# josebeo2016/SCL-Deepfake-audio-detection

Hardware: AMD Instinct MI355X
Metric: train-step utterances/sec (64000-sample clips) (higher is better)
Workload: dtype bf16

## Files before the change

### scl-deepfake-audio-detection_amd/csrc/gemm.hip

```cpp
#include "gemm_common.h"

using namespace sclg;

namespace {

constexpr int BM = 128, BN = 128;

struct StageK {
    __amdgpu_buffer_rsrc_t rsrc;
    unsigned rowoff[4];
    unsigned lds_off[4];
    int kcur, kend;

    __device__ __forceinline__ void init(const OpK& o, const char* base, int row0, int rowlimit, int kbegin, int kend_, int tid) {
        rsrc = make_rsrc(base);
        const int c = tid & 7;
#pragma unroll
        for (int i = 0; i < 4; ++i) {
            const int row = (tid >> 3) + 32 * i;
            const int r = row0 + row;
            rowoff[i] = r < rowlimit ? row_off(o, (unsigned)r) : OOB;
            lds_off[i] = (unsigned)(row * 128 + ((c ^ ((row >> 1) & 7)) << 4));
        }
        kcur = kbegin + 8 * c; kend = kend_;
// ... 817 lines not shown
}

extern "C" int scl_gemm_bf16(const SclGemmDesc* dp, void* stream) {
    SCL_REQUIRE(dp, "gemm: null desc");
    const SclGemmDesc& d = *dp;
    GemmK k;
    {
        const int rc = gemm_fill_k(d, k);
        if (rc != SCL_OK) return rc;
    }
    const bool at = d.flags & SCL_GEMM_A_T, bt = d.flags & SCL_GEMM_B_T;
    const bool f32ab = d.flags & SCL_GEMM_AB_F32;
    const int tiles = ((d.M + BM - 1) / BM) * ((d.N + BN - 1) / BN);
    const long long zdim = (long long)d.nb1 * d.nb2 * d.splitk;
    dim3 grid(tiles, 1, (unsigned)zdim), block(256);
    const size_t lds = 4 * TILE_BYTES;
    hipStream_t s = (hipStream_t)stream;
    if (f32ab) {
        SclProfScope prof(SCL_KID_GEMM_F32, s, 2.0 * d.M * d.N * (double)d.K * d.nb1 * d.nb2, true);
        const int rc = scl_gemm_f32_launch(d, k, s);
        if (rc != SCL_OK) return rc;
        return scl_check_launch("scl_gemm_bf16(f32 operands)");
    }
    {
        SclProfScope prof(SCL_KID_GEMM, s, 2.0 * d.M * d.N * (double)d.K * d.nb1 * d.nb2, true);
        const bool a_whole = at ? (d.M % 8 == 0) : (d.K % 8 == 0);
        const bool b_whole = bt ? (d.N % 8 == 0) : (d.K % 8 == 0);
        const bool dma = a_whole && b_whole && !(d.flags & SCL_GEMM_NO_DMA);
#ifdef SCL_EXPERIMENTS
        const long long big_tiles = (long long)((d.M + BIG_BM - 1) / BIG_BM) * ((d.N + BN - 1) / BN) * zdim;
        const bool big = dma && (d.flags & SCL_GEMM_FORCE_BIG) && !(d.flags & SCL_GEMM_NO_BIG) && d.M >= 256 && d.K >= 192 && big_tiles >= 1;
        const long long p8_tiles = (long long)((d.M + P8_BM - 1) / P8_BM) * ((d.N + P8_BN - 1) / P8_BN) * zdim;
        const bool p8 = dma && (d.flags & SCL_GEMM_FORCE_P8) && !(d.flags & SCL_GEMM_NO_P8);
#else
        const bool big = false, p8 = false;
#endif
        W8Plan plan;
#ifdef SCL_EXPERIMENTS
        const bool x2 = dma && gemm_pick_x2(k, at, bt, d, zdim, &plan);
#else
        const bool x2 = false;
#endif
        const bool w8 = !x2 && dma && gemm_pick_w8(k, at, bt, d, zdim, &plan);
        if (((unsigned)d.flags & SCL_GEMM_C_SPLIT3) && !w8) {
            scl_set_error("gemm: C_SPLIT3 is served by the wide-tile kernel only, and this launch (M %d, N %d, K %d) does not qualify for it", d.M, d.N, d.K);
            return SCL_EUNSUPPORTED;
        }
#ifdef SCL_EXPERIMENTS
        const char* deep_env = getenv("SCL_GEMM_DEEP");
        const bool deep = !x2 && !w8 && dma && deep_env && atoi(deep_env) != 0 && (long long)tiles * zdim <= 256 && (d.K + BK - 1) / BK / d.splitk >= 4;
#else
        const bool deep = false;
#endif
        prof.note(d.M, d.N, d.K, d.flags, (int)zdim, x2 ? 3 : (w8 ? (plan.variant == 2 ? 6 : 1 + plan.variant) : (deep ? 7 : 0)));
        if (x2) {
#ifdef SCL_EXPERIMENTS
            scl_gemm_x2_launch(k, at, bt, plan, zdim, s);
#endif
        } else if (w8) {
            scl_gemm_w8_launch(k, at, bt, plan, zdim, s);
#ifdef SCL_EXPERIMENTS
        } else if (p8) {
            static bool p8_attr_set = false;
            if (!p8_attr_set) {
                hipFuncSetAttribute((const void*)scl_gemm_p8_kernel<false, false>, hipFuncAttributeMaxDynamicSharedMemorySize, P8_LDS);
                hipFuncSetAttribute((const void*)scl_gemm_p8_kernel<false, true>, hipFuncAttributeMaxDynamicSharedMemorySize, P8_LDS);
                hipFuncSetAttribute((const void*)scl_gemm_p8_kernel<true, false>, hipFuncAttributeMaxDynamicSharedMemorySize, P8_LDS);
                hipFuncSetAttribute((const void*)scl_gemm_p8_kernel<true, true>, hipFuncAttributeMaxDynamicSharedMemorySize, P8_LDS);
                p8_attr_set = true;
            }
            dim3 pgrid((unsigned)(p8_tiles / zdim), 1, (unsigned)zdim), pblock(512);
            if (!at && !bt) SCL_LAUNCH((scl_gemm_p8_kernel<false, false>), pgrid, pblock, P8_LDS, s, k);
            else if (!at && bt) SCL_LAUNCH((scl_gemm_p8_kernel<false, true>), pgrid, pblock, P8_LDS, s, k);
            else if (at && !bt) SCL_LAUNCH((scl_gemm_p8_kernel<true, false>), pgrid, pblock, P8_LDS, s, k);
            else SCL_LAUNCH((scl_gemm_p8_kernel<true, true>), pgrid, pblock, P8_LDS, s, k);
        } else if (big) {
            static bool attr_set = false;
            if (!attr_set) {
                hipFuncSetAttribute((const void*)scl_gemm_big_kernel<false, false>, hipFuncAttributeMaxDynamicSharedMemorySize, BIG_LDS);
                hipFuncSetAttribute((const void*)scl_gemm_big_kernel<false, true>, hipFuncAttributeMaxDynamicSharedMemorySize, BIG_LDS);
                hipFuncSetAttribute((const void*)scl_gemm_big_kernel<true, false>, hipFuncAttributeMaxDynamicSharedMemorySize, BIG_LDS);
                hipFuncSetAttribute((const void*)scl_gemm_big_kernel<true, true>, hipFuncAttributeMaxDynamicSharedMemorySize, BIG_LDS);
                attr_set = true;
            }
            dim3 bgrid(((d.M + BIG_BM - 1) / BIG_BM) * ((d.N + BN - 1) / BN), 1, (unsigned)zdim), bblock(512);
            if (!at && !bt) SCL_LAUNCH((scl_gemm_big_kernel<false, false>), bgrid, bblock, BIG_LDS, s, k);
            else if (!at && bt) SCL_LAUNCH((scl_gemm_big_kernel<false, true>), bgrid, bblock, BIG_LDS, s, k);
            else if (at && !bt) SCL_LAUNCH((scl_gemm_big_kernel<true, false>), bgrid, bblock, BIG_LDS, s, k);
            else SCL_LAUNCH((scl_gemm_big_kernel<true, true>), bgrid, bblock, BIG_LDS, s, k);
#endif
#ifdef SCL_EXPERIMENTS
        } else if (deep) {
            static bool deep_attr_set = false;
            if (!deep_attr_set) {
                hipFuncSetAttribute((const void*)scl_gemm_deep_kernel<false, false, DEEP_S>, hipFuncAttributeMaxDynamicSharedMemorySize, DEEP_LDS);
                hipFuncSetAttribute((const void*)scl_gemm_deep_kernel<false, true, DEEP_S>, hipFuncAttributeMaxDynamicSharedMemorySize, DEEP_LDS);
                hipFuncSetAttribute((const void*)scl_gemm_deep_kernel<true, false, DEEP_S>, hipFuncAttributeMaxDynamicSharedMemorySize, DEEP_LDS);
                hipFuncSetAttribute((const void*)scl_gemm_deep_kernel<true, true, DEEP_S>, hipFuncAttributeMaxDynamicSharedMemorySize, DEEP_LDS);
                deep_attr_set = true;
            }
            if (!at && !bt) SCL_LAUNCH((scl_gemm_deep_kernel<false, false, DEEP_S>), grid, block, DEEP_LDS, s, k);
            else if (!at && bt) SCL_LAUNCH((scl_gemm_deep_kernel<false, true, DEEP_S>), grid, block, DEEP_LDS, s, k);
            else if (at && !bt) SCL_LAUNCH((scl_gemm_deep_kernel<true, false, DEEP_S>), grid, block, DEEP_LDS, s, k);
            else SCL_LAUNCH((scl_gemm_deep_kernel<true, true, DEEP_S>), grid, block, DEEP_LDS, s, k);
#endif
        } else if (dma) {
            if (!at && !bt) SCL_LAUNCH((scl_gemm_dma_kernel<false, false>), grid, block, lds, s, k);
// ... 118 lines not shown
```

### scl-deepfake-audio-detection_amd/csrc/gemm_common.h

```cpp
#pragma once
#include "common.h"

namespace sclg {

constexpr int BK = 64;
constexpr int TILE_BYTES = 128 * 64 * 2;
constexpr unsigned OOB = 0xFFFFFFFFu;

struct OpK {
    const void* ptr;
    long long bs1, bs2;
    unsigned rb_bytes, ld_bytes, cout_bytes;
    unsigned rpb, rpb_magic, rpb_shift;
    unsigned cin, cin_magic, cin_mshift, esz_shift;
};
struct GemmK {
    OpK A, B;
    void* C; void* C2; const void* R; const float* bias; float* colsum;
    long long c_bs1, c_bs2, c_rbstride, c_split_stride, bias_bs2;
    unsigned c_rpb, c_magic, c_shift;
    int ldc, M, N, K, nb2, splitk, flags, vec_ok, group_m, tile_m, debug;
    float alpha, drop_p;
    unsigned drop_seed;
};
// ... 206 lines not shown
                    v[0] *= act_grad_f(ract, r0); v[1] *= act_grad_f(ract, r1); v[2] *= act_grad_f(ract, r2); v[3] *= act_grad_f(ract, r3);
                }
                if (drop) {
                    v[0] *= dropout_scale(d.drop_seed, (uint64_t)(off + 0), d.drop_p); v[1] *= dropout_scale(d.drop_seed, (uint64_t)(off + 1), d.drop_p);
                    v[2] *= dropout_scale(d.drop_seed, (uint64_t)(off + 2), d.drop_p); v[3] *= dropout_scale(d.drop_seed, (uint64_t)(off + 3), d.drop_p);
                }
                if (rmode == 1) { v[0] += r0; v[1] += r1; v[2] += r2; v[3] += r3; }
                if (c_f32) *reinterpret_cast<float4*>(reinterpret_cast<float*>(d.C) + off) = make_float4(v[0], v[1], v[2], v[3]);
                else *reinterpret_cast<uint2*>(reinterpret_cast<bf16_t*>(d.C) + off) = make_uint2(pack_bf2(v[0], v[1]), pack_bf2(v[2], v[3]));
            } else if (rok) {
                epi_scalar(ea, v[0], off + 0, col + 0, bias);
                epi_scalar(ea, v[1], off + 1, col + 1, bias);
                epi_scalar(ea, v[2], off + 2, col + 2, bias);
                epi_scalar(ea, v[3], off + 3, col + 3, bias);
            }
        }
        }
    }
}

template <int NMT>
__device__ __forceinline__ void gemm_epilogue_blk(const GemmK& d, f32x4 (&acc)[NMT][4], int mbase, int nbase, int mlimit, int nmt,
                                                  int z1, int z2, int ksplit, int lane) {
    constexpr int KEY = SCL_GEMM_C_F32 | SCL_GEMM_C2_F32 | SCL_GEMM_R_F32 | SCL_GEMM_HAS_BIAS | SCL_GEMM_HAS_C2 | SCL_GEMM_DROPOUT |
                        (0xF << SCL_GEMM_ACT_SHIFT) | (0xF << SCL_GEMM_RMODE_SHIFT) | (0xF << SCL_GEMM_RACT_SHIFT);
    const int f = d.flags & KEY, fb = f & ~SCL_GEMM_HAS_BIAS;
    if (!(d.debug & 16)) {
        if (fb == 0) return gemm_epilogue_blk_k<NMT, 1>(d, acc, mbase, nbase, mlimit, nmt, z1, z2, ksplit, lane);
        if (f == (SCL_GEMM_HAS_BIAS | SCL_GEMM_HAS_C2 | (5 << SCL_GEMM_ACT_SHIFT))) return gemm_epilogue_blk_k<NMT, 2>(d, acc, mbase, nbase, mlimit, nmt, z1, z2, ksplit, lane);
        if (f == ((2 << SCL_GEMM_RMODE_SHIFT) | (4 << SCL_GEMM_RACT_SHIFT))) return gemm_epilogue_blk_k<NMT, 3>(d, acc, mbase, nbase, mlimit, nmt, z1, z2, ksplit, lane);
        if (fb == (SCL_GEMM_C_F32 | SCL_GEMM_R_F32 | (1 << SCL_GEMM_RMODE_SHIFT))) return gemm_epilogue_blk_k<NMT, 4>(d, acc, mbase, nbase, mlimit, nmt, z1, z2, ksplit, lane);
        if (fb == SCL_GEMM_C_F32) return gemm_epilogue_blk_k<NMT, 5>(d, acc, mbase, nbase, mlimit, nmt, z1, z2, ksplit, lane);
    }
    gemm_epilogue_blk_k<NMT, 0>(d, acc, mbase, nbase, mlimit, nmt, z1, z2, ksplit, lane);
}

__device__ __forceinline__ void gemm_epilogue(const GemmK& d, f32x4 (&acc)[4][4], int m0, int n0, int z1, int z2, int ksplit,
                                              int lane, int wr, int wc) {
    gemm_epilogue_blk<4>(d, acc, m0 + wr * 64, n0 + wc * 64, d.M, 4, z1, z2, ksplit, lane);
}





void make_magic(unsigned dv, unsigned* magic, unsigned* shift);
bool fill_operand(const SclOperand& o, const char* name, long long rows, long long contig, OpK* k, int esz);
int scl_gemm_f32_launch(const SclGemmDesc& d, GemmK& k, hipStream_t s);

struct W8Plan { int variant, tiles_m, tile_m; long long tiles, cost; int ncu = 0; };
bool scl_gemm_w8_plan(const GemmK& k, bool at, bool bt, const SclGemmDesc& d, long long zdim, int ncu, W8Plan* plan);
int scl_gemm_read_stamps(unsigned long long* out, int nblocks);
long long scl_gemm_w8p_launches();
int scl_gemm_w8_launch(GemmK& k, bool at, bool bt, const W8Plan& plan, long long zdim, hipStream_t s);
constexpr int W8_GROUP_MAX = 8;
bool scl_gemm_w8_group_member_ok(const GemmK& k, bool at, bool bt, const SclGemmDesc& d);
int scl_gemm_w8_group_tiles(const GemmK& k);
int scl_gemm_w8_group_launch(GemmK* ks, int n, const int* tile0, const int* ntile, hipStream_t s);

bool scl_gemm_x2_plan(const GemmK& k, bool at, bool bt, const SclGemmDesc& d, long long zdim, int ncu, W8Plan* plan);
int scl_gemm_x2_launch(GemmK& k, bool at, bool bt, const W8Plan& plan, long long zdim, hipStream_t s);

}
```

### scl-deepfake-audio-detection_amd/csrc/gemm_w8.hip

```cpp
#include "gemm_common.h"
#include "gemm_w8_epi.h"

using namespace sclg;

__device__ unsigned long long scl_gemm_stamps[4096 * 8];

namespace {

__device__ __forceinline__ void w8_stamp(const GemmK& d, int slot, int lane, int wave) {
    if ((d.flags & SCL_GEMM_STAMPS) && wave == 0 && lane == 0 && blockIdx.x < 4096 && blockIdx.z == 0) {
        scl_gemm_stamps[blockIdx.x * 8 + 2 * slot] = __builtin_amdgcn_s_memrealtime();
        scl_gemm_stamps[blockIdx.x * 8 + 2 * slot + 1] = __builtin_amdgcn_s_memtime();
    }
}

constexpr int W8_BN = 256;
constexpr int W8_OPB = 2 * TILE_BYTES;
constexpr int W8_NA = 3, W8_NB = 2;
constexpr int W8_LDS = (W8_NA + W8_NB) * W8_OPB;

struct W8K {
    __amdgpu_buffer_rsrc_t rsrc;
    unsigned voff[4];
    __device__ __forceinline__ void init(const OpK& o, const char* base, int row0, int rowlimit, int lane, int wave) {
// ... 414 lines not shown
    lb.template issue2<0>(smem + W8_NA * W8_OPB, wave, soffB, nk > 0); lb.template issue2<2>(smem + W8_NA * W8_OPB, wave, soffB, nk > 0);
    soffA += stepA; soffB += stepB;
    la.template issue2<0>(smem + W8_OPB, wave, soffA, nk > 1); la.template issue2<2>(smem + W8_OPB, wave, soffA, nk > 1);
    lb.template issue2<0>(smem + (W8_NA + 1) * W8_OPB, wave, soffB, nk > 1); lb.template issue2<2>(smem + (W8_NA + 1) * W8_OPB, wave, soffB, nk > 1);
    asm volatile("s_waitcnt vmcnt(8)" ::: "memory");
    w8_stamp(d, 1, lane, wave);
    __builtin_amdgcn_s_barrier();
    if (RB0 == RB1) {
        w8s_body<AT, BT, RB0>(d, smem, la, lb, nk, soffA, soffB, wr * RB0, m0, n0, mlimit, z1, z2, ksplit, lane, wave, wc);
    } else if (wr == 0) {
        w8s_body<AT, BT, RB0>(d, smem, la, lb, nk, soffA, soffB, 0, m0, n0, mlimit, z1, z2, ksplit, lane, wave, wc);
    } else {
        w8s_body<AT, BT, RB1>(d, smem, la, lb, nk, soffA, soffB, RB0, m0, n0, mlimit, z1, z2, ksplit, lane, wave, wc);
    }
}

template <bool AT, bool BT, int RB0, int RB1>
__global__ __launch_bounds__(512, 2) void scl_gemm_w8s_kernel(const GemmK d) {
    extern __shared__ __attribute__((aligned(16))) char smem[];
    w8s_tile<AT, BT, RB0, RB1>(d, smem, blockIdx.x, gridDim.x, blockIdx.z);
}

struct GemmGroupK {
    GemmK k[W8_GROUP_MAX];
    int first[W8_GROUP_MAX + 1];
    int tile0[W8_GROUP_MAX];
    int ntiles[W8_GROUP_MAX];
    int n;
    int xcd_major;
};
typedef const __attribute__((address_space(4))) GemmGroupK* W8GArg;
template <bool AT, bool BT, int RB0, int RB1>
__global__ __launch_bounds__(512, 2) void scl_gemm_w8s_group_kernel(const GemmGroupK g) {
    extern __shared__ __attribute__((aligned(16))) char smem[];
    W8GArg gp = (W8GArg)__builtin_amdgcn_kernarg_segment_ptr();
    const int total = g.first[W8_GROUP_MAX];
    const int x = blockIdx.x & 7, idx = blockIdx.x >> 3, q = total >> 3, r = total & 7;
#ifdef SCL_EXPERIMENTS
    const int pos = (g.xcd_major ? ((x < r ? x * (q + 1) : r * (q + 1) + (x - r) * q) + idx) : (int)blockIdx.x);
#else
    const int pos = (x < r ? x * (q + 1) : r * (q + 1) + (x - r) * q) + idx;
#endif
    int mem = 0;
#pragma unroll
    for (int i = 1; i < W8_GROUP_MAX; ++i) mem += (i < g.n && pos >= g.first[i]) ? 1 : 0;
    mem = __builtin_amdgcn_readfirstlane(mem);
    const int t = __builtin_amdgcn_readfirstlane(pos - gp->first[mem] + gp->tile0[mem]);
#ifdef SCL_EXPERIMENTS
    if (!g.xcd_major) { w8s_tile<AT, BT, RB0, RB1, false>(*(const GemmK*)&gp->k[mem], smem, t, gp->ntiles[mem], 0); return; }
#endif
    w8s_tile<AT, BT, RB0, RB1, true>(*(const GemmK*)&gp->k[mem], smem, t, gp->ntiles[mem], 0);
}

#ifdef SCL_EXPERIMENTS
typedef const __attribute__((address_space(4))) GemmK* W8KArg;
__device__ __forceinline__ const GemmK* w8p_args(W8KArg p) {
    asm volatile("" : "+s"(p));
    return (const GemmK*)p;
}
template <bool AT, bool BT, int RBW>
__device__ __forceinline__ void w8p_body(const GemmK& d, W8KArg kp, char* smem, const char* Ab, const char* Bb, int ab, int tiles_m, int tiles_n,
                                         int lane, int wave, int wc) {
    typedef typename W8Sel<AT>::type LA;
    typedef typename W8Sel<BT>::type LB;
    const unsigned stepA = LA::kstep(d.A), stepB = LB::kstep(d.B);
    const int nk = d.K / BK;
    const int ntiles = tiles_m * tiles_n, G = gridDim.x;
    const int nbk = wc * 4;
    char* const bimg = smem + W8_NA * W8_OPB;
    char *a_cur = smem, *a_nxt = smem + W8_OPB, *a_fill = smem + 2 * W8_OPB;
    int bpar = 0;
    int v = blockIdx.x, tm, tn;
    tile_coords(v, ntiles, tiles_m, tiles_n, tm, tn, d.group_m);
    const int tile_m = d.tile_m, Mrows = d.M, group_m = d.group_m;
    int m0 = tm * tile_m, n0 = tn * W8_BN, mlimit = min(Mrows, m0 + tile_m);
    LA la;
    LB lb;
    la.init(d.A, Ab, m0, mlimit, lane, wave);
    lb.init(d.B, Bb, n0, d.N, lane, wave);
    la.set_batched(false); lb.set_batched(false);
    la.template issue2<0>(a_cur, wave, 0u, true); la.template issue2<2>(a_cur, wave, 0u, true);
    lb.template issue2<0>(bimg, wave, 0u, true); lb.template issue2<2>(bimg, wave, 0u, true);
    la.template issue2<0>(a_nxt, wave, stepA, true); la.template issue2<2>(a_nxt, wave, stepA, true);
    lb.template issue2<0>(bimg + W8_OPB, wave, stepB, true); lb.template issue2<2>(bimg + W8_OPB, wave, stepB, true);
    asm volatile("s_waitcnt vmcnt(8)" ::: "memory");
    __builtin_amdgcn_s_barrier();
#define W8S_READ(FA, FB, TA, TB, KS)                                                        \
    _Pragma("unroll") for (int j = 0; j < 4; ++j) FB[j] = w8_frag<BT>(TB, nbk + j, KS, lane); \
    _Pragma("unroll") for (int i = 0; i < RBW; ++i) FA[i] = w8_frag<AT>(TA, ab + i, KS, lane);
#define W8S_MFMA(FA, FB)                                                                    \
    _Pragma("unroll") for (int i = 0; i < RBW; ++i)                                         \
        _Pragma("unroll") for (int j = 0; j < 4; ++j)                                       \
            acc[i][j] = __builtin_amdgcn_mfma_f32_16x16x32_bf16(FB[j], FA[i], acc[i][j], 0, 0, 0);
    for (;;) {
        f32x4 acc[RBW][4];
#pragma unroll
        for (int i = 0; i < RBW; ++i)
#pragma unroll
            for (int j = 0; j < 4; ++j) acc[i][j] = f32x4{0.f, 0.f, 0.f, 0.f};
        bf16x8 fa0[RBW], fa1[RBW], fb0[4], fb1[4];
        const int vn = v + G;
        const bool has_next = vn < ntiles;
        int m0n = 0, n0n = 0, mlimn = 0;
        if (has_next) {
            tile_coords(vn, ntiles, tiles_m, tiles_n, tm, tn, group_m);
            m0n = tm * tile_m; n0n = tn * W8_BN; mlimn = min(Mrows, m0n + tile_m);
        }
        unsigned soffA = stepA, soffB = stepB;
        W8S_READ(fa0, fb0, a_cur, bimg + bpar * W8_OPB, 0)
        for (int kt = 0; kt < nk; ++kt) {
            char* tB = bimg + ((kt + bpar) & 1) * W8_OPB;
            const bool hand = kt + 2 == nk;
            const bool live2 = kt + 2 < nk || (hand && has_next);
            soffA += stepA; soffB += stepB;
            asm volatile("s_waitcnt lgkmcnt(0)" ::: "memory");
            __builtin_amdgcn_sched_barrier(0);
            W8S_READ(fa1, fb1, a_cur, tB, 1)
            __builtin_amdgcn_sched_barrier(0);
            W8S_MFMA(fa0, fb0)
            __builtin_amdgcn_sched_barrier(0);
            if (hand && has_next) {
                const GemmK* dh = w8p_args(kp);
                la.init(dh->A, reinterpret_cast<const char*>(dh->A.ptr), m0n, mlimn, lane, wave);
            }
            {
                const unsigned sa = hand ? 0u : soffA;
                la.template issue2<0>(a_fill, wave, sa, live2); la.template issue2<2>(a_fill, wave, sa, live2);
            }
            asm volatile("s_waitcnt lgkmcnt(0)" ::: "memory");
            asm volatile("s_waitcnt vmcnt(4)" ::: "memory");
            __builtin_amdgcn_sched_barrier(0);
            __builtin_amdgcn_s_barrier();
            __builtin_amdgcn_sched_barrier(0);
            if (hand && has_next) {
                const GemmK* dh = w8p_args(kp);
                lb.init(dh->B, reinterpret_cast<const char*>(dh->B.ptr), n0n, dh->N, lane, wave);
            }
            {
                const unsigned sb = hand ? 0u : soffB;
                lb.template issue2<0>(tB, wave, sb, live2); lb.template issue2<2>(tB, wave, sb, live2);
            }
            if (kt + 1 < nk) { W8S_READ(fa0, fb0, a_nxt, bimg + (((kt + bpar) & 1) ^ 1) * W8_OPB, 0) }
            __builtin_amdgcn_sched_barrier(0);
            W8S_MFMA(fa1, fb1)
            __builtin_amdgcn_sched_barrier(0);
            char* t = a_cur; a_cur = a_nxt; a_nxt = a_fill; a_fill = t;
        }
        asm volatile("s_waitcnt vmcnt(0)" ::: "memory");
        asm volatile("s_waitcnt lgkmcnt(0)" ::: "memory");
        __builtin_amdgcn_s_barrier();
        char* const bfree = bimg + ((nk - 1 + bpar) & 1) * W8_OPB;
        {
            const GemmK& d = *w8p_args(kp);
            const float* bias = (d.flags & SCL_GEMM_HAS_BIAS) ? d.bias : nullptr;
            char* wlds = a_fill + wave * 4096;
            const int bstride = (int)(a_nxt - a_fill);
            char* wextra = bfree + wave * 4096;
            float* cs0 = d.colsum ? d.colsum + ((long long)(m0 / tile_m) * 4 + (wave >> 2) * 2) * d.N : nullptr;
            float cs[8];
#pragma unroll
            for (int pr = 0; pr < (RBW + 1) / 2; ++pr) {
                if (pr == 0 || pr == 2) {
#pragma unroll
                    for (int j = 0; j < 8; ++j) cs[j] = 0.f;
                }
                if (2 * pr + 1 < RBW) {
                    f32x4 (&a2)[2][4] = *reinterpret_cast<f32x4 (*)[2][4]>(&acc[2 * pr]);
                    w8_epilogue_pass<2, 0>(d, a2, 2, wlds, wextra, m0 + (ab + 2 * pr) * 16, n0 + wc * 64, mlimit, 0ll, bias, lane, nullptr,
                                        cs0 ? cs : nullptr, bstride);
                } else {
                    f32x4 (&a1)[1][4] = *reinterpret_cast<f32x4 (*)[1][4]>(&acc[2 * pr]);
                    w8_epilogue_pass<1, 0>(d, a1, 1, wlds, wextra, m0 + (ab + 2 * pr) * 16, n0 + wc * 64, mlimit, 0ll, bias, lane, nullptr,
                                        cs0 ? cs : nullptr, bstride);
                }
                if (cs0 && (pr == 1 || pr == (RBW + 1) / 2 - 1)) w8_colsum_store(d, cs, cs0 + (pr >> 1) * d.N, n0 + wc * 64, lane);
            }
        }
        if (!has_next) break;
        asm volatile("s_waitcnt lgkmcnt(0)" ::: "memory");
        __builtin_amdgcn_sched_barrier(0);
        la.template issue2<0>(a_nxt, wave, stepA, true); la.template issue2<2>(a_nxt, wave, stepA, true);
        lb.template issue2<0>(bfree, wave, stepB, true); lb.template issue2<2>(bfree, wave, stepB, true);
        bpar = (bpar + nk) & 1;
        v = vn; m0 = m0n; n0 = n0n; mlimit = mlimn;
    }
#undef W8S_READ
#undef W8S_MFMA
}

template <bool AT, bool BT, int RB0, int RB1>
__global__ __launch_bounds__(512, 2) void scl_gemm_w8p_kernel(const GemmK d) {
    extern __shared__ __attribute__((aligned(16))) char smem[];
    const int tid = threadIdx.x, lane = tid & 63;
    const int wave = __builtin_amdgcn_readfirstlane(tid >> 6);
    const int wr = wave >> 2, wc = wave & 3;
    const int tiles_m = (d.M + d.tile_m - 1) / d.tile_m, tiles_n = (d.N + W8_BN - 1) / W8_BN;
    const char* Ab = reinterpret_cast<const char*>(d.A.ptr);
    const char* Bb = reinterpret_cast<const char*>(d.B.ptr);
    W8KArg kp = (W8KArg)__builtin_amdgcn_kernarg_segment_ptr();
    if (RB0 == RB1) {
        w8p_body<AT, BT, RB0>(d, kp, smem, Ab, Bb, wr * RB0, tiles_m, tiles_n, lane, wave, wc);
    } else if (wr == 0) {
        w8p_body<AT, BT, RB0>(d, kp, smem, Ab, Bb, 0, tiles_m, tiles_n, lane, wave, wc);
    } else {
        w8p_body<AT, BT, RB1>(d, kp, smem, Ab, Bb, RB0, tiles_m, tiles_n, lane, wave, wc);
    }
}

#endif

template <int RB0, int RB1>
void w8_launch_rb(const GemmK& k, bool at, bool bt, dim3 grid, hipStream_t s, int mode) {
    static bool attr_set = false;
    if (!attr_set) {
        (void)hipFuncSetAttribute((const void*)scl_gemm_w8_kernel<false, false, RB0, RB1>, hipFuncAttributeMaxDynamicSharedMemorySize, W8_LDS);
        (void)hipFuncSetAttribute((const void*)scl_gemm_w8_kernel<false, true, RB0, RB1>, hipFuncAttributeMaxDynamicSharedMemorySize, W8_LDS);
        (void)hipFuncSetAttribute((const void*)scl_gemm_w8_kernel<true, false, RB0, RB1>, hipFuncAttributeMaxDynamicSharedMemorySize, W8_LDS);
        (void)hipFuncSetAttribute((const void*)scl_gemm_w8_kernel<true, true, RB0, RB1>, hipFuncAttributeMaxDynamicSharedMemorySize, W8_LDS);
        (void)hipFuncSetAttribute((const void*)scl_gemm_w8s_kernel<false, false, RB0, RB1>, hipFuncAttributeMaxDynamicSharedMemorySize, W8_LDS);
        (void)hipFuncSetAttribute((const void*)scl_gemm_w8s_kernel<false, true, RB0, RB1>, hipFuncAttributeMaxDynamicSharedMemorySize, W8_LDS);
        (void)hipFuncSetAttribute((const void*)scl_gemm_w8s_kernel<true, false, RB0, RB1>, hipFuncAttributeMaxDynamicSharedMemorySize, W8_LDS);
        (void)hipFuncSetAttribute((const void*)scl_gemm_w8s_kernel<true, true, RB0, RB1>, hipFuncAttributeMaxDynamicSharedMemorySize, W8_LDS);
#ifdef SCL_EXPERIMENTS
        if constexpr (RB0 == 7) {
            (void)hipFuncSetAttribute((const void*)scl_gemm_w8p_kernel<false, false, RB0, RB1>, hipFuncAttributeMaxDynamicSharedMemorySize, W8_LDS);
            (void)hipFuncSetAttribute((const void*)scl_gemm_w8p_kernel<false, true, RB0, RB1>, hipFuncAttributeMaxDynamicSharedMemorySize, W8_LDS);
            (void)hipFuncSetAttribute((const void*)scl_gemm_w8p_kernel<true, false, RB0, RB1>, hipFuncAttributeMaxDynamicSharedMemorySize, W8_LDS);
        }
#endif
        attr_set = true;
    }
    const dim3 block(512);
#ifdef SCL_EXPERIMENTS
    if constexpr (RB0 == 7) {
        if (mode == 2) {
            if (!at && !bt) SCL_LAUNCH((scl_gemm_w8p_kernel<false, false, RB0, RB1>), grid, block, W8_LDS, s, k);
            else if (!at && bt) SCL_LAUNCH((scl_gemm_w8p_kernel<false, true, RB0, RB1>), grid, block, W8_LDS, s, k);
            else SCL_LAUNCH((scl_gemm_w8p_kernel<true, false, RB0, RB1>), grid, block, W8_LDS, s, k);
            return;
        }
    }
#endif
    if (mode == 1) {
        if (!at && !bt) SCL_LAUNCH((scl_gemm_w8s_kernel<false, false, RB0, RB1>), grid, block, W8_LDS, s, k);
        else if (!at && bt) SCL_LAUNCH((scl_gemm_w8s_kernel<false, true, RB0, RB1>), grid, block, W8_LDS, s, k);
        else if (at && !bt) SCL_LAUNCH((scl_gemm_w8s_kernel<true, false, RB0, RB1>), grid, block, W8_LDS, s, k);
        else SCL_LAUNCH((scl_gemm_w8s_kernel<true, true, RB0, RB1>), grid, block, W8_LDS, s, k);
        return;
    }
    if (!at && !bt) SCL_LAUNCH((scl_gemm_w8_kernel<false, false, RB0, RB1>), grid, block, W8_LDS, s, k);
    else if (!at && bt) SCL_LAUNCH((scl_gemm_w8_kernel<false, true, RB0, RB1>), grid, block, W8_LDS, s, k);
    else if (at && !bt) SCL_LAUNCH((scl_gemm_w8_kernel<true, false, RB0, RB1>), grid, block, W8_LDS, s, k);
    else SCL_LAUNCH((scl_gemm_w8_kernel<true, true, RB0, RB1>), grid, block, W8_LDS, s, k);
}

void w8_launch_43(const GemmK& k, bool bt, dim3 grid, hipStream_t s) {
    static bool attr_set = false;
    if (!attr_set) {
        (void)hipFuncSetAttribute((const void*)scl_gemm_w8s_kernel<false, false, 4, 3>, hipFuncAttributeMaxDynamicSharedMemorySize, W8_LDS);
        (void)hipFuncSetAttribute((const void*)scl_gemm_w8s_kernel<false, true, 4, 3>, hipFuncAttributeMaxDynamicSharedMemorySize, W8_LDS);
        attr_set = true;
    }
    if (!bt) SCL_LAUNCH((scl_gemm_w8s_kernel<false, false, 4, 3>), grid, dim3(512), W8_LDS, s, k);
    else SCL_LAUNCH((scl_gemm_w8s_kernel<false, true, 4, 3>), grid, dim3(512), W8_LDS, s, k);
}

}

namespace sclg {

bool scl_gemm_w8_plan(const GemmK& k, bool at, bool bt, const SclGemmDesc& d, long long zdim, int ncu, W8Plan* plan) {
    auto flat_rows = [](const SclOperand& o, long long rows) { return (long long)o.rpb >= rows; };
    const bool tt = at && bt;
    const bool a_ok = at ? (flat_rows(d.A, d.K) || (tt && d.A.rpb >= 1)) : (d.A.cin == 0x7fffffff || d.A.cin == 64 || d.A.cin >= d.K);
    const bool b_ok = bt ? (flat_rows(d.B, d.K) || (tt && d.B.rpb >= 1)) : (d.B.cin == 0x7fffffff || d.B.cin == 64 || d.B.cin >= d.K);
    if (!a_ok || !b_ok || (d.K % BK) != 0) return false;
    const long long tiles_n = (d.N + W8_BN - 1) / W8_BN;
    long long best = -1;
    const char* e43 = getenv("SCL_W8_TILE112");
    const char* epp = getenv("SCL_W8_MODE");
    const bool v43_env = !e43 || atoi(e43) != 0, pingpong_env = epp && *epp && atoi(epp) == 0;
    const bool v43_ok = v43_env && !pingpong_env && !at && zdim == 1 && !d.colsum_part && !(d.flags & SCL_GEMM_STAMPS);
    for (int v = 0; v < (v43_ok ? 3 : 2); ++v) {
        const int bm = v == 0 ? 208 : (v == 1 ? 256 : 112);
        const long long ntm = (d.M + bm - 1) / bm;
        const long long rounds = (ntm * tiles_n * zdim + ncu - 1) / ncu;
        const long long cost = rounds * (bm + W8_BN);
        if (best < 0 || cost < best) {
            best = cost;
            plan->variant = v; plan->tiles_m = (int)ntm; plan->tile_m = (int)((d.M + ntm - 1) / ntm);
            plan->tiles = ntm * tiles_n; plan->cost = cost; plan->ncu = ncu;
        }
    }
    return true;
}

bool scl_gemm_w8_group_member_ok(const GemmK& k, bool at, bool bt, const SclGemmDesc& d) {
    if (!at || !bt || d.nb1 != 1 || d.nb2 != 1 || d.splitk != 1 || (d.K % BK) != 0 || d.K / BK < 3) return false;
    if ((long long)d.A.rpb < (long long)d.K || (long long)d.B.rpb < (long long)d.K) return false;
    if ((d.M % 8) || (d.N % 8) || !k.vec_ok) return false;
    const int plain = SCL_GEMM_A_T | SCL_GEMM_B_T | SCL_GEMM_C_F32;
    return (d.flags & ~(SCL_GEMM_NO_DMA | SCL_GEMM_NO_W8)) == plain && !d.colsum_part;
}

int scl_gemm_w8_group_tiles(const GemmK& k) { return ((k.M + 255) / 256) * ((k.N + W8_BN - 1) / W8_BN); }

int scl_gemm_w8_group_launch(GemmK* ks, int n, const int* tile0, const int* ntile, hipStream_t s) {
    GemmGroupK g = GemmGroupK();
    int total = 0;
    for (int i = 0; i < n; ++i) {
        GemmK& k = ks[i];
        const int ntm = (k.M + 255) / 256;
        k.tile_m = (k.M + ntm - 1) / ntm;
        k.debug = 0;
        g.k[i] = k;
        g.first[i] = total;
        g.ntiles[i] = scl_gemm_w8_group_tiles(k);
        g.tile0[i] = tile0 ? tile0[i] : 0;
        total += ntile ? ntile[i] : g.ntiles[i];
    }
    for (int i = n; i <= W8_GROUP_MAX; ++i) g.first[i] = total;
    g.n = n;
#ifdef SCL_EXPERIMENTS
    static const int xcd_major = [] { const char* e = getenv("SCL_WGRAD_XCD_MAJOR"); return e ? atoi(e) : 1; }();
    g.xcd_major = xcd_major;
#else
    g.xcd_major = 1;
#endif
    static bool attr_set = false;
    if (!attr_set) {
        (void)hipFuncSetAttribute((const void*)scl_gemm_w8s_group_kernel<true, true, 8, 8>, hipFuncAttributeMaxDynamicSharedMemorySize, W8_LDS);
        attr_set = true;
    }
    SCL_LAUNCH((scl_gemm_w8s_group_kernel<true, true, 8, 8>), dim3((unsigned)total), dim3(512), W8_LDS, s, g);
    return 0;
}

static long long w8p_launches = 0;
long long scl_gemm_w8p_launches() { return w8p_launches; }

int scl_gemm_read_stamps(unsigned long long* out, int nblocks) {
    return hipMemcpyFromSymbol(out, HIP_SYMBOL(scl_gemm_stamps), sizeof(unsigned long long) * 8 * (size_t)nblocks) == hipSuccess ? 0 : -1;
}

int scl_gemm_w8_launch(GemmK& k, bool at, bool bt, const W8Plan& plan, long long zdim, hipStream_t s) {
    k.tile_m = plan.tile_m;
    k.debug = 0;
    {
        const long long nb1 = zdim / ((long long)k.nb2 * k.splitk);
        const long long rows = k.M - 1, rpb = (long long)k.c_rpb;
        const long long maxoff = (nb1 - 1) * k.c_bs1 + ((long long)k.nb2 - 1) * k.c_bs2 + (rows / rpb) * k.c_rbstride + (rows % rpb) * k.ldc + k.N;
        if (maxoff * ((k.flags & SCL_GEMM_R_F32) ? 4 : 2) >= 0xFFFFFF00ll) k.debug |= 2;
    }
    const dim3 grid((unsigned)plan.tiles, 1, (unsigned)zdim);
    const char* me = getenv("SCL_W8_MODE");
    int mode = (me && *me) ? atoi(me) : 1;
    if (at && bt) {
        if ((long long)k.A.rpb < (long long)k.K) { k.debug |= 4; mode = 0; }
        if ((long long)k.B.rpb < (long long)k.K) { k.debug |= 8; mode = 0; }
    }
    {
        static const bool epi_generic = [] { const char* e = getenv("SCL_W8_EPI_GENERIC"); return e && atoi(e) != 0; }();
        if (epi_generic) k.debug |= 16;
    }
    dim3 g = grid;
#ifdef SCL_EXPERIMENTS
    {
        const char* sg = getenv("SCL_W8_STAGGER");
        const int stg = sg ? atoi(sg) : 0;
        if (stg > 0 && plan.tiles > 256 && zdim == 1) k.debug |= (stg & 0xFF) << 8;
    }
    const char* pe = getenv("SCL_GEMM_PERSIST");
    const int pv = pe ? atoi(pe) : 0;
    if (mode == 1 && pv > 0 && !(at && bt) && zdim == 1 && k.splitk == 1 && k.K / BK >= 3 && !(k.flags & SCL_GEMM_STAMPS)) {
        const long long ncu = plan.ncu >= 8 ? plan.ncu : 256;
        const long long rounds = (plan.tiles + ncu - 1) / ncu;
        long long G = pv >= 8 ? (pv & ~7) : ((((plan.tiles + rounds - 1) / rounds) + 7) & ~7ll);
        if (G > (ncu & ~7ll) && pv < 8) G = ncu & ~7ll;
        if (plan.variant == 0 && (pv >= 8 || rounds >= 2) && G >= 8 && G < plan.tiles) { mode = 2; g = dim3((unsigned)G, 1, 1); ++w8p_launches; }
    }
#endif
    if (plan.variant == 2) w8_launch_43(k, bt, g, s);
    else if (plan.variant == 0) w8_launch_rb<7, 6>(k, at, bt, g, s, mode);
    else w8_launch_rb<8, 8>(k, at, bt, g, s, mode);
    return 0;
}

}
```

Baseline: 1593.

## Enable persistent wide-tile GEMM kernel by default with interleaved LDS reads and epilogue specialization

Moves the persistent (grid-stride over output tiles) wide-tile GEMM kernel out of the experimental build and makes it the default whenever the tile count is at least twice the chosen grid size. The main loop now interleaves LDS fragment reads, MFMA groups and per-chunk global loads with fine-grained LDS wait counts instead of full lgkmcnt(0) waits. Next-tile address setup overlaps the last K iterations, and the epilogue is specialized at compile time per flag pattern. The aim is to cut tail-wave and launch-fill overhead and hide load latency, at the cost of more kernel variants, a narrower set of eligible shapes, and a risk of scheduling regressions for shapes it now captures.

```diff
diff --git a/scl-deepfake-audio-detection_amd/csrc/gemm.hip b/scl-deepfake-audio-detection_amd/csrc/gemm.hip
--- a/scl-deepfake-audio-detection_amd/csrc/gemm.hip
+++ b/scl-deepfake-audio-detection_amd/csrc/gemm.hip
@@ -893,7 +893,8 @@
 #else
         const bool deep = false;
 #endif
-        prof.note(d.M, d.N, d.K, d.flags, (int)zdim, x2 ? 3 : (w8 ? (plan.variant == 2 ? 6 : 1 + plan.variant) : (deep ? 7 : 0)));
+        const bool w8p = w8 && scl_gemm_w8_persist_blocks(k, at, bt, plan, zdim) > 0;
+        prof.note(d.M, d.N, d.K, d.flags, (int)zdim, x2 ? 3 : (w8p ? 8 : (w8 ? (plan.variant == 2 ? 6 : 1 + plan.variant) : (deep ? 7 : 0))));
         if (x2) {
 #ifdef SCL_EXPERIMENTS
             scl_gemm_x2_launch(k, at, bt, plan, zdim, s);
diff --git a/scl-deepfake-audio-detection_amd/csrc/gemm_common.h b/scl-deepfake-audio-detection_amd/csrc/gemm_common.h
--- a/scl-deepfake-audio-detection_amd/csrc/gemm_common.h
+++ b/scl-deepfake-audio-detection_amd/csrc/gemm_common.h
@@ -282,6 +282,7 @@
 bool scl_gemm_w8_plan(const GemmK& k, bool at, bool bt, const SclGemmDesc& d, long long zdim, int ncu, W8Plan* plan);
 int scl_gemm_read_stamps(unsigned long long* out, int nblocks);
 long long scl_gemm_w8p_launches();
+int scl_gemm_w8_persist_blocks(const GemmK& k, bool at, bool bt, const W8Plan& plan, long long zdim);
 int scl_gemm_w8_launch(GemmK& k, bool at, bool bt, const W8Plan& plan, long long zdim, hipStream_t s);
 constexpr int W8_GROUP_MAX = 8;
 bool scl_gemm_w8_group_member_ok(const GemmK& k, bool at, bool bt, const SclGemmDesc& d);
diff --git a/scl-deepfake-audio-detection_amd/csrc/gemm_w8.hip b/scl-deepfake-audio-detection_amd/csrc/gemm_w8.hip
--- a/scl-deepfake-audio-detection_amd/csrc/gemm_w8.hip
+++ b/scl-deepfake-audio-detection_amd/csrc/gemm_w8.hip
@@ -490,46 +490,68 @@
     w8s_tile<AT, BT, RB0, RB1, true>(*(const GemmK*)&gp->k[mem], smem, t, gp->ntiles[mem], 0);
 }
 
-#ifdef SCL_EXPERIMENTS
 typedef const __attribute__((address_space(4))) GemmK* W8KArg;
 __device__ __forceinline__ const GemmK* w8p_args(W8KArg p) {
     asm volatile("" : "+s"(p));
     return (const GemmK*)p;
 }
-template <bool AT, bool BT, int RBW>
-__device__ __forceinline__ void w8p_body(const GemmK& d, W8KArg kp, char* smem, const char* Ab, const char* Bb, int ab, int tiles_m, int tiles_n,
-                                         int lane, int wave, int wc) {
+__device__ __forceinline__ int w8p_lane() {
+    int l = (int)__builtin_amdgcn_mbcnt_hi(~0u, __builtin_amdgcn_mbcnt_lo(~0u, 0u));
+    asm volatile("" : "+v"(l));
+    return l;
+}
+constexpr int W8_EPI_KEY = SCL_GEMM_C_F32 | SCL_GEMM_C2_F32 | SCL_GEMM_R_F32 | SCL_GEMM_HAS_BIAS | SCL_GEMM_HAS_C2 | SCL_GEMM_DROPOUT |
+                           (0xF << SCL_GEMM_ACT_SHIFT) | (0xF << SCL_GEMM_RMODE_SHIFT) | (0xF << SCL_GEMM_RACT_SHIFT);
+inline int w8p_epi_kind(int flags) {
+    const int f = flags & W8_EPI_KEY, fb = f & ~SCL_GEMM_HAS_BIAS;
+    if (fb == 0) return 1;
+    if (f == (SCL_GEMM_HAS_BIAS | SCL_GEMM_HAS_C2 | (5 << SCL_GEMM_ACT_SHIFT))) return 2;
+    if (fb == SCL_GEMM_C_F32) return 5;
+    return 0;
+}
+
+template <bool AT, bool BT, int RBW, int EK>
+__device__ __forceinline__ void w8p_body(W8KArg kp, char* smem, const int ab, const int lane, const int wave, const int wc) {
     typedef typename W8Sel<AT>::type LA;
     typedef typename W8Sel<BT>::type LB;
-    const unsigned stepA = LA::kstep(d.A), stepB = LB::kstep(d.B);
-    const int nk = d.K / BK;
-    const int ntiles = tiles_m * tiles_n, G = gridDim.x;
+    typedef W8SRead<AT, BT, RBW> RD;
+    constexpr int NRD = RBW + 4, OPA = AT ? 2 : 1, OPB = BT ? 2 : 1;
+    constexpr int RQ0 = 4, RQ1 = 8, RQ2 = NRD;
+    static_assert(RBW >= 6 && RBW <= 8, "w8p_body: 6 to 8 row blocks per wave");
+    auto ops_upto = [](int n) constexpr { return (n > 0 ? OPB : 0) + (n > 1 ? (n - 1 < RBW ? n - 1 : RBW) * OPA : 0) + (n > RBW + 1 ? (n - RBW - 1) * OPB : 0); };
     const int nbk = wc * 4;
     char* const bimg = smem + W8_NA * W8_OPB;
     char *a_cur = smem, *a_nxt = smem + W8_OPB, *a_fill = smem + 2 * W8_OPB;
-    int bpar = 0;
-    int v = blockIdx.x, tm, tn;
-    tile_coords(v, ntiles, tiles_m, tiles_n, tm, tn, d.group_m);
-    const int tile_m = d.tile_m, Mrows = d.M, group_m = d.group_m;
-    int m0 = tm * tile_m, n0 = tn * W8_BN, mlimit = min(Mrows, m0 + tile_m);
     LA la;
     LB lb;
-    la.init(d.A, Ab, m0, mlimit, lane, wave);
-    lb.init(d.B, Bb, n0, d.N, lane, wave);
     la.set_batched(false); lb.set_batched(false);
+    int nk, tile_m, Mrows, group_m, tiles_m, tiles_n, m0, n0, mlimit;
+    unsigned stepA, stepB;
+    int v = blockIdx.x;
+    {
+        const GemmK* d0 = w8p_args(kp);
+        nk = d0->K / BK;
+        tile_m = d0->tile_m; Mrows = d0->M; group_m = d0->group_m;
+        tiles_m = __builtin_amdgcn_readfirstlane((Mrows + tile_m - 1) / tile_m);
+        tiles_n = (d0->N + W8_BN - 1) / W8_BN;
+        if (v >= tiles_m * tiles_n) return;
+        stepA = LA::kstep(d0->A); stepB = LB::kstep(d0->B);
+        int tm, tn;
+        tile_coords(v, tiles_m * tiles_n, tiles_m, tiles_n, tm, tn, group_m);
+        m0 = tm * tile_m; n0 = tn * W8_BN; mlimit = min(Mrows, m0 + tile_m);
+        la.init(d0->A, reinterpret_cast<const char*>(d0->A.ptr), m0, mlimit, lane, wave);
+        lb.init(d0->B, reinterpret_cast<const char*>(d0->B.ptr), n0, d0->N, lane, wave);
+    }
+    const int ntiles = tiles_m * tiles_n, G = gridDim.x;
     la.template issue2<0>(a_cur, wave, 0u, true); la.template issue2<2>(a_cur, wave, 0u, true);
     lb.template issue2<0>(bimg, wave, 0u, true); lb.template issue2<2>(bimg, wave, 0u, true);
     la.template issue2<0>(a_nxt, wave, stepA, true); la.template issue2<2>(a_nxt, wave, stepA, true);
     lb.template issue2<0>(bimg + W8_OPB, wave, stepB, true); lb.template issue2<2>(bimg + W8_OPB, wave, stepB, true);
     asm volatile("s_waitcnt vmcnt(8)" ::: "memory");
     __builtin_amdgcn_s_barrier();
-#define W8S_READ(FA, FB, TA, TB, KS)                                                        \
-    _Pragma("unroll") for (int j = 0; j < 4; ++j) FB[j] = w8_frag<BT>(TB, nbk + j, KS, lane); \
-    _Pragma("unroll") for (int i = 0; i < RBW; ++i) FA[i] = w8_frag<AT>(TA, ab + i, KS, lane);
-#define W8S_MFMA(FA, FB)                                                                    \
-    _Pragma("unroll") for (int i = 0; i < RBW; ++i)                                         \
-        _Pragma("unroll") for (int j = 0; j < 4; ++j)                                       \
-            acc[i][j] = __builtin_amdgcn_mfma_f32_16x16x32_bf16(FB[j], FA[i], acc[i][j], 0, 0, 0);
+    int bpar = 0;
+    unsigned soffA = stepA, soffB = stepB;
+    int m0n = 0, n0n = 0, mlimn = 0;
     for (;;) {
         f32x4 acc[RBW][4];
 #pragma unroll
@@ -537,115 +559,125 @@
 #pragma unroll
             for (int j = 0; j < 4; ++j) acc[i][j] = f32x4{0.f, 0.f, 0.f, 0.f};
         bf16x8 fa0[RBW], fa1[RBW], fb0[4], fb1[4];
-        const int vn = v + G;
-        const bool has_next = vn < ntiles;
-        int m0n = 0, n0n = 0, mlimn = 0;
-        if (has_next) {
-            tile_coords(vn, ntiles, tiles_m, tiles_n, tm, tn, group_m);
-            m0n = tm * tile_m; n0n = tn * W8_BN; mlimn = min(Mrows, m0n + tile_m);
-        }
-        unsigned soffA = stepA, soffB = stepB;
-        W8S_READ(fa0, fb0, a_cur, bimg + bpar * W8_OPB, 0)
+        const bool has_next = v + G < ntiles;
+        lds_wait_upto(0);
+        __builtin_amdgcn_sched_barrier(0);
+        RD::template go<0, NRD, true>(fa0, fb0, a_cur, bimg + bpar * W8_OPB, ab, nbk, 0, lane);
         for (int kt = 0; kt < nk; ++kt) {
             char* tB = bimg + ((kt + bpar) & 1) * W8_OPB;
-            const bool hand = kt + 2 == nk;
-            const bool live2 = kt + 2 < nk || (hand && has_next);
+            const bool live2 = kt + 2 < nk || has_next;
             soffA += stepA; soffB += stepB;
-            asm volatile("s_waitcnt lgkmcnt(0)" ::: "memory");
+            if (kt + 2 == nk) {
+                soffA = 0u; soffB = 0u;
+                if (has_next) {
+                    int tm, tn;
+                    tile_coords(v + G, ntiles, tiles_m, tiles_n, tm, tn, group_m);
+                    m0n = tm * tile_m; n0n = tn * W8_BN; mlimn = min(Mrows, m0n + tile_m);
+                    const GemmK* dh = w8p_args(kp);
+                    const int ln = w8p_lane();
+                    la.init(dh->A, reinterpret_cast<const char*>(dh->A.ptr), m0n, mlimn, ln, wave);
+                    lb.init(dh->B, reinterpret_cast<const char*>(dh->B.ptr), n0n, dh->N, ln, wave);
+                    lds_wait_upto(0);
+                    __builtin_amdgcn_sched_barrier(0);
+                }
+            }
+#define W8P_Q_FIRST(j, R0, R1)                                                                                               \
+            RD::template go<R0, R1, false>(fa1, fb1, a_cur, tB, ab, nbk, 1, lane);                                           \
+            __builtin_amdgcn_sched_barrier(0);                                                                               \
+            lds_wait_upto((3 - (j)) * OPB + ops_upto(R1));                                                                   \
+            __builtin_amdgcn_sched_barrier(0);                                                                               \
+            _Pragma("unroll") for (int i = 0; i < RBW; ++i)                                                                  \
+                acc[i][j] = __builtin_amdgcn_mfma_f32_16x16x32_bf16(fb0[j], fa0[i], acc[i][j], 0, 0, 0);                     \
+            __builtin_amdgcn_sched_barrier(0);                                                                               \
+            la.issue1(a_fill, wave, soffA, live2, j);                                                                        \
             __builtin_amdgcn_sched_barrier(0);
-            W8S_READ(fa1, fb1, a_cur, tB, 1)
-            __builtin_amdgcn_sched_barrier(0);
-            W8S_MFMA(fa0, fb0)
-            __builtin_amdgcn_sched_barrier(0);
-            if (hand && has_next) {
-                const GemmK* dh = w8p_args(kp);
-                la.init(dh->A, reinterpret_cast<const char*>(dh->A.ptr), m0n, mlimn, lane, wave);
-            }
-            {
-                const unsigned sa = hand ? 0u : soffA;
-                la.template issue2<0>(a_fill, wave, sa, live2); la.template issue2<2>(a_fill, wave, sa, live2);
-            }
-            asm volatile("s_waitcnt lgkmcnt(0)" ::: "memory");
+            W8P_Q_FIRST(0, 0, RQ0) W8P_Q_FIRST(1, RQ0, RQ1) W8P_Q_FIRST(2, RQ1, RQ2) W8P_Q_FIRST(3, RQ2, NRD)
+#undef W8P_Q_FIRST
+            lds_wait_upto(0);
             asm volatile("s_waitcnt vmcnt(4)" ::: "memory");
             __builtin_amdgcn_sched_barrier(0);
             __builtin_amdgcn_s_barrier();
             __builtin_amdgcn_sched_barrier(0);
-            if (hand && has_next) {
-                const GemmK* dh = w8p_args(kp);
-                lb.init(dh->B, reinterpret_cast<const char*>(dh->B.ptr), n0n, dh->N, lane, wave);
-            }
-            {
-                const unsigned sb = hand ? 0u : soffB;
-                lb.template issue2<0>(tB, wave, sb, live2); lb.template issue2<2>(tB, wave, sb, live2);
-            }
-            if (kt + 1 < nk) { W8S_READ(fa0, fb0, a_nxt, bimg + (((kt + bpar) & 1) ^ 1) * W8_OPB, 0) }
+            const char* tBn = bimg + (((kt + bpar) & 1) ^ 1) * W8_OPB;
+#define W8P_B_ISSUE(j) if ((j) < 2) { lb.issue1(tB, wave, soffB, live2, 2 * (j)); lb.issue1(tB, wave, soffB, live2, 2 * (j) + 1); }
+#define W8P_Q_SECOND(j, R0, R1)                                                                                              \
+            RD::template go<R0, R1, false>(fa0, fb0, a_nxt, tBn, ab, nbk, 0, lane);                                          \
+            __builtin_amdgcn_sched_barrier(0);                                                                               \
+            _Pragma("unroll") for (int i = 0; i < RBW; ++i)                                                                  \
+                acc[i][j] = __builtin_amdgcn_mfma_f32_16x16x32_bf16(fb1[j], fa1[i], acc[i][j], 0, 0, 0);                     \
+            __builtin_amdgcn_sched_barrier(0);                                                                               \
+            W8P_B_ISSUE(j)                                                                                                   \
             __builtin_amdgcn_sched_barrier(0);
-            W8S_MFMA(fa1, fb1)
-            __builtin_amdgcn_sched_barrier(0);
+            W8P_Q_SECOND(0, 0, RQ0) W8P_Q_SECOND(1, RQ0, RQ1) W8P_Q_SECOND(2, RQ1, RQ2) W8P_Q_SECOND(3, RQ2, NRD)
+#undef W8P_Q_SECOND
+#undef W8P_B_ISSUE
             char* t = a_cur; a_cur = a_nxt; a_nxt = a_fill; a_fill = t;
         }
-        asm volatile("s_waitcnt vmcnt(0)" ::: "memory");
-        asm volatile("s_waitcnt lgkmcnt(0)" ::: "memory");
-        __builtin_amdgcn_s_barrier();
-        char* const bfree = bimg + ((nk - 1 + bpar) & 1) * W8_OPB;
+        lds_wait_upto(0);
+        __builtin_amdgcn_sched_barrier(0);
         {
             const GemmK& d = *w8p_args(kp);
-            const float* bias = (d.flags & SCL_GEMM_HAS_BIAS) ? d.bias : nullptr;
+            const int ln = w8p_lane();
+            const float* bias = (EK == 2 || (d.flags & SCL_GEMM_HAS_BIAS)) ? d.bias : nullptr;
             char* wlds = a_fill + wave * 4096;
-            const int bstride = (int)(a_nxt - a_fill);
-            char* wextra = bfree + wave * 4096;
             float* cs0 = d.colsum ? d.colsum + ((long long)(m0 / tile_m) * 4 + (wave >> 2) * 2) * d.N : nullptr;
             float cs[8];
 #pragma unroll
-            for (int pr = 0; pr < (RBW + 1) / 2; ++pr) {
-                if (pr == 0 || pr == 2) {
+            for (int b = 0; b < RBW; ++b) {
+                if (b == 0 || b == 4) {
 #pragma unroll
                     for (int j = 0; j < 8; ++j) cs[j] = 0.f;
                 }
-                if (2 * pr + 1 < RBW) {
-                    f32x4 (&a2)[2][4] = *reinterpret_cast<f32x4 (*)[2][4]>(&acc[2 * pr]);
-                    w8_epilogue_pass<2, 0>(d, a2, 2, wlds, wextra, m0 + (ab + 2 * pr) * 16, n0 + wc * 64, mlimit, 0ll, bias, lane, nullptr,
-                                        cs0 ? cs : nullptr, bstride);
-                } else {
-                    f32x4 (&a1)[1][4] = *reinterpret_cast<f32x4 (*)[1][4]>(&acc[2 * pr]);
-                    w8_epilogue_pass<1, 0>(d, a1, 1, wlds, wextra, m0 + (ab + 2 * pr) * 16, n0 + wc * 64, mlimit, 0ll, bias, lane, nullptr,
-                                        cs0 ? cs : nullptr, bstride);
-                }
-                if (cs0 && (pr == 1 || pr == (RBW + 1) / 2 - 1)) w8_colsum_store(d, cs, cs0 + (pr >> 1) * d.N, n0 + wc * 64, lane);
+                f32x4 (&a1)[1][4] = *reinterpret_cast<f32x4 (*)[1][4]>(&acc[b]);
+                w8_epilogue_pass_k<1, EK>(d, a1, 1, wlds, wlds, m0 + (ab + b) * 16, n0 + wc * 64, mlimit, 0ll, bias, ln, nullptr, cs, 4096);
+                if (cs0 && (b == 3 || b == RBW - 1)) w8_colsum_store(d, cs, cs0 + (b >> 2) * d.N, n0 + wc * 64, ln);
             }
         }
         if (!has_next) break;
-        asm volatile("s_waitcnt lgkmcnt(0)" ::: "memory");
-        __builtin_amdgcn_sched_barrier(0);
-        la.template issue2<0>(a_nxt, wave, stepA, true); la.template issue2<2>(a_nxt, wave, stepA, true);
-        lb.template issue2<0>(bfree, wave, stepB, true); lb.template issue2<2>(bfree, wave, stepB, true);
         bpar = (bpar + nk) & 1;
-        v = vn; m0 = m0n; n0 = n0n; mlimit = mlimn;
-    }
-#undef W8S_READ
-#undef W8S_MFMA
-}
-
-template <bool AT, bool BT, int RB0, int RB1>
-__global__ __launch_bounds__(512, 2) void scl_gemm_w8p_kernel(const GemmK d) {
+        v += G; m0 = m0n; n0 = n0n; mlimit = mlimn;
+    }
+}
+
+template <bool AT, bool BT, int EK, int RB0, int RB1>
+__global__ __launch_bounds__(512, 2) void scl_gemm_persist_w8_kernel(const GemmK d) {
     extern __shared__ __attribute__((aligned(16))) char smem[];
     const int tid = threadIdx.x, lane = tid & 63;
     const int wave = __builtin_amdgcn_readfirstlane(tid >> 6);
-    const int wr = wave >> 2, wc = wave & 3;
-    const int tiles_m = (d.M + d.tile_m - 1) / d.tile_m, tiles_n = (d.N + W8_BN - 1) / W8_BN;
-    const char* Ab = reinterpret_cast<const char*>(d.A.ptr);
-    const char* Bb = reinterpret_cast<const char*>(d.B.ptr);
     W8KArg kp = (W8KArg)__builtin_amdgcn_kernarg_segment_ptr();
-    if (RB0 == RB1) {
-        w8p_body<AT, BT, RB0>(d, kp, smem, Ab, Bb, wr * RB0, tiles_m, tiles_n, lane, wave, wc);
-    } else if (wr == 0) {
-        w8p_body<AT, BT, RB0>(d, kp, smem, Ab, Bb, 0, tiles_m, tiles_n, lane, wave, wc);
+    if (RB0 == RB1) w8p_body<AT, BT, RB0, EK>(kp, smem, (wave >> 2) * RB0, lane, wave, wave & 3);
+    else if ((wave >> 2) == 0) w8p_body<AT, BT, RB0, EK>(kp, smem, 0, lane, wave, wave & 3);
+    else w8p_body<AT, BT, RB1, EK>(kp, smem, RB0, lane, wave, wave & 3);
+}
+
+template <bool AT, bool BT, int EK, int RB0, int RB1>
+void w8p_launch_k(const GemmK& k, dim3 grid, hipStream_t s) {
+    static bool attr_set = false;
+    if (!attr_set) {
+        (void)hipFuncSetAttribute((const void*)scl_gemm_persist_w8_kernel<AT, BT, EK, RB0, RB1>, hipFuncAttributeMaxDynamicSharedMemorySize, W8_LDS);
+        attr_set = true;
+    }
+    SCL_LAUNCH((scl_gemm_persist_w8_kernel<AT, BT, EK, RB0, RB1>), grid, dim3(512), W8_LDS, s, k);
+}
+bool w8p_built(bool bt, int ek, int variant) {
+    if (variant == 0) return ek == 1 || ek == 2 || ek == 5;
+    return variant == 1 && ((!bt && ek == 5) || (bt && ek == 1));
+}
+void w8p_launch(const GemmK& k, bool bt, int ek, int variant, dim3 grid, hipStream_t s) {
+    if (variant == 1) {
+        if (!bt) w8p_launch_k<false, false, 5, 8, 8>(k, grid, s);
+        else w8p_launch_k<false, true, 1, 8, 8>(k, grid, s);
+    } else if (!bt) {
+        if (ek == 1) w8p_launch_k<false, false, 1, 7, 6>(k, grid, s);
+        else if (ek == 2) w8p_launch_k<false, false, 2, 7, 6>(k, grid, s);
+        else w8p_launch_k<false, false, 5, 7, 6>(k, grid, s);
     } else {
-        w8p_body<AT, BT, RB1>(d, kp, smem, Ab, Bb, RB0, tiles_m, tiles_n, lane, wave, wc);
-    }
-}
-
-#endif
+        if (ek == 1) w8p_launch_k<false, true, 1, 7, 6>(k, grid, s);
+        else if (ek == 2) w8p_launch_k<false, true, 2, 7, 6>(k, grid, s);
+        else w8p_launch_k<false, true, 5, 7, 6>(k, grid, s);
+    }
+}
+
 
 template <int RB0, int RB1>
 void w8_launch_rb(const GemmK& k, bool at, bool bt, dim3 grid, hipStream_t s, int mode) {
@@ -659,26 +691,9 @@
         (void)hipFuncSetAttribute((const void*)scl_gemm_w8s_kernel<false, true, RB0, RB1>, hipFuncAttributeMaxDynamicSharedMemorySize, W8_LDS);
         (void)hipFuncSetAttribute((const void*)scl_gemm_w8s_kernel<true, false, RB0, RB1>, hipFuncAttributeMaxDynamicSharedMemorySize, W8_LDS);
         (void)hipFuncSetAttribute((const void*)scl_gemm_w8s_kernel<true, true, RB0, RB1>, hipFuncAttributeMaxDynamicSharedMemorySize, W8_LDS);
-#ifdef SCL_EXPERIMENTS
-        if constexpr (RB0 == 7) {
-            (void)hipFuncSetAttribute((const void*)scl_gemm_w8p_kernel<false, false, RB0, RB1>, hipFuncAttributeMaxDynamicSharedMemorySize, W8_LDS);
-            (void)hipFuncSetAttribute((const void*)scl_gemm_w8p_kernel<false, true, RB0, RB1>, hipFuncAttributeMaxDynamicSharedMemorySize, W8_LDS);
-            (void)hipFuncSetAttribute((const void*)scl_gemm_w8p_kernel<true, false, RB0, RB1>, hipFuncAttributeMaxDynamicSharedMemorySize, W8_LDS);
-        }
-#endif
         attr_set = true;
     }
     const dim3 block(512);
-#ifdef SCL_EXPERIMENTS
-    if constexpr (RB0 == 7) {
-        if (mode == 2) {
-            if (!at && !bt) SCL_LAUNCH((scl_gemm_w8p_kernel<false, false, RB0, RB1>), grid, block, W8_LDS, s, k);
-            else if (!at && bt) SCL_LAUNCH((scl_gemm_w8p_kernel<false, true, RB0, RB1>), grid, block, W8_LDS, s, k);
-            else SCL_LAUNCH((scl_gemm_w8p_kernel<true, false, RB0, RB1>), grid, block, W8_LDS, s, k);
-            return;
-        }
-    }
-#endif
     if (mode == 1) {
         if (!at && !bt) SCL_LAUNCH((scl_gemm_w8s_kernel<false, false, RB0, RB1>), grid, block, W8_LDS, s, k);
         else if (!at && bt) SCL_LAUNCH((scl_gemm_w8s_kernel<false, true, RB0, RB1>), grid, block, W8_LDS, s, k);
@@ -781,6 +796,23 @@
     return hipMemcpyFromSymbol(out, HIP_SYMBOL(scl_gemm_stamps), sizeof(unsigned long long) * 8 * (size_t)nblocks) == hipSuccess ? 0 : -1;
 }
 
+int scl_gemm_w8_persist_blocks(const GemmK& k, bool at, bool bt, const W8Plan& plan, long long zdim) {
+    const char* pe = getenv("SCL_W8_PERSIST");
+    const int pv = (pe && *pe) ? atoi(pe) : 1;
+    const char* me = getenv("SCL_W8_MODE");
+    static const bool epi_generic = [] { const char* e = getenv("SCL_W8_EPI_GENERIC"); return e && atoi(e) != 0; }();
+    if (pv <= 0 || (me && *me && atoi(me) != 1) || epi_generic) return 0;
+    if (plan.variant > 1 || at || zdim != 1 || k.splitk != 1 || k.K / BK < 3 || (k.flags & SCL_GEMM_STAMPS)) return 0;
+    const int ek = w8p_epi_kind(k.flags);
+    if (!ek || !w8p_built(bt, ek, plan.variant) || ((unsigned)k.flags & SCL_GEMM_C_SPLIT3) || !k.vec_ok || (k.ldc & 7) || (k.c_rbstride & 7)) return 0;
+    if (pv >= 8) return pv > 256 ? 256 : (pv & ~7);
+    const long long ncu = plan.ncu >= 8 ? plan.ncu : 256;
+    const long long rounds = (plan.tiles + ncu - 1) / ncu;
+    long long G = (((plan.tiles + rounds - 1) / rounds) + 7) & ~7ll;
+    if (G > (ncu & ~7ll)) G = ncu & ~7ll;
+    return (G >= 8 && plan.tiles >= 2 * G) ? (int)G : 0;
+}
+
 int scl_gemm_w8_launch(GemmK& k, bool at, bool bt, const W8Plan& plan, long long zdim, hipStream_t s) {
     k.tile_m = plan.tile_m;
     k.debug = 0;
@@ -808,16 +840,15 @@
         const int stg = sg ? atoi(sg) : 0;
         if (stg > 0 && plan.tiles > 256 && zdim == 1) k.debug |= (stg & 0xFF) << 8;
     }
-    const char* pe = getenv("SCL_GEMM_PERSIST");
-    const int pv = pe ? atoi(pe) : 0;
-    if (mode == 1 && pv > 0 && !(at && bt) && zdim == 1 && k.splitk == 1 && k.K / BK >= 3 && !(k.flags & SCL_GEMM_STAMPS)) {
-        const long long ncu = plan.ncu >= 8 ? plan.ncu : 256;
-        const long long rounds = (plan.tiles + ncu - 1) / ncu;
-        long long G = pv >= 8 ? (pv & ~7) : ((((plan.tiles + rounds - 1) / rounds) + 7) & ~7ll);
-        if (G > (ncu & ~7ll) && pv < 8) G = ncu & ~7ll;
-        if (plan.variant == 0 && (pv >= 8 || rounds >= 2) && G >= 8 && G < plan.tiles) { mode = 2; g = dim3((unsigned)G, 1, 1); ++w8p_launches; }
-    }
 #endif
+    if (mode == 1) {
+        const int G = scl_gemm_w8_persist_blocks(k, at, bt, plan, zdim);
+        if (G > 0) {
+            ++w8p_launches;
+            w8p_launch(k, bt, w8p_epi_kind(k.flags), plan.variant, dim3((unsigned)G, 1, 1), s);
+            return 0;
+        }
+    }
     if (plan.variant == 2) w8_launch_43(k, bt, g, s);
     else if (plan.variant == 0) w8_launch_rb<7, 6>(k, at, bt, g, s, mode);
     else w8_launch_rb<8, 8>(k, at, bt, g, s, mode);
```

Result: faster. 1621 (median of 6 runs) (+1.8%).
